# daigo0927/tf-raft

Hardware: AMD Instinct MI355X
Metric: image-pairs/sec at 448×512 iters_pred=24; final-iter EPE vs TF ref (higher is better)
Workload: dtype f32; 1 GPU; RAFT forward BASELINE configs[1]: batch 4/GPU 448x512 iters_pred=24 random weights; pairs_per_gpu=4, global_batch=4, parallelism=dp1, collective=none

## Files before the change

### include/raft_hip.h

```cpp
#ifndef RAFT_HIP_H_
#define RAFT_HIP_H_

#include <stddef.h>
#include <stdint.h>

#ifdef __cplusplus
extern "C" {
#endif

#define RAFT_HIP_VERSION 222
#define RAFT_MAX_LEVELS 4

enum {
    RAFT_OK = 0,
    RAFT_E_NULL = -1,
    RAFT_E_SHAPE = -2,
    RAFT_E_UNSUPPORTED = -3,
    RAFT_E_ALIGN = -4
};

int raft_version(void);
const char *raft_error_string(int rc);

int raft_set_option(const char *name, const char *value);
int raft_set_thread_concurrency(int n);
int raft_get_option(const char *name, char *buf, size_t len);

uint32_t raft_crc32c(uint32_t crc, const void *data, size_t n);


int raft_corr_pyramid_layout(int B, int h, int w, int levels,
                             int64_t *level_offsets ,
                             int *lh , int *lw );

int64_t raft_corr_build_workspace_floats(int B, int h, int w, int C, int levels);

int raft_corr_build_f32(const float *fmap1, const float *fmap2, int B, int h, int w, int C,
                        int levels, float *pyr, const int64_t *level_offsets,
                        float *workspace, void *stream);

int raft_corr_lookup_f32(const float *pyr, const int64_t *level_offsets, const float *coords,
                         int B, int h, int w, int levels, int radius,
                         float *out, int ld_out, void *stream);

int raft_fmap_pyramid_f32(const float *fmap2, int B, int h, int w, int C, int levels,
                          float *fmap2_pyr, void *stream);
int raft_corr_lookup_ondemand_f32(const float *fmap1, const float *fmap2_pyr,
                                  const float *coords, int B, int h, int w, int C,
                                  int levels, int radius, float *out, int ld_out,
                                  void *stream);

int raft_bilinear_sampler_f32(const float *image, const float *coords, int64_t n, int h, int w,
                              int kh, int kw, float *out, void *stream);

int raft_coords_grid_f32(float *coords, int B, int h, int w, void *stream);


int raft_upsample_convex_f32(const float *flow, const float *mask, int B, int h, int w,
                             float *out, void *stream);

int raft_upflow8_f32(const float *flow, int B, int h, int w, float *out, void *stream);

int raft_stream_copy_f32(const float *src, float *dst, int64_t n, void *stream);

int raft_crop_or_pad_f32(const float *src, float *dst, int N, int Hs, int Ws, int Ht, int Wt, int C, void *stream);
int raft_crop_or_pad_u8_f32(const uint8_t *src, float *dst, int N, int Hs, int Ws, int Ht, int Wt, int C, void *stream);
int raft_crop_or_pad_u8(const uint8_t *src, uint8_t *dst, int N, int Hs, int Ws, int Ht, int Wt, int C, void *stream);

int raft_resize_f32(const float *src, float *dst, int N, int Hs, int Ws, int Ht, int Wt, int C,
                    const int *y_first, const int *y_count, const float *y_weights, int y_max_taps,
                    const int *x_first, const int *x_count, const float *x_weights, int x_max_taps,
                    const float *chan_scale, void *stream);
int raft_resize_u8_f32(const uint8_t *src, float *dst, int N, int Hs, int Ws, int Ht, int Wt, int C,
                       const int *y_first, const int *y_count, const float *y_weights, int y_max_taps,
                       const int *x_first, const int *x_count, const float *x_weights, int x_max_taps,
                       const float *chan_scale, void *stream);

#define RAFT_TILE_MAX_PER_AXIS 32
#define RAFT_TILE_MAX_TAPS 4
typedef struct RaftTileOrigins {
    int32_t ny, nx;
    int32_t oy[RAFT_TILE_MAX_PER_AXIS];
    int32_t ox[RAFT_TILE_MAX_PER_AXIS];
} RaftTileOrigins;

int raft_tile_gather_f32(const float *src, float *dst, int N, int Hs, int Ws, int Ht, int Wt, int C, RaftTileOrigins origins,
                         void *stream);
int raft_tile_gather_u8_f32(const uint8_t *src, float *dst, int N, int Hs, int Ws, int Ht, int Wt, int C, RaftTileOrigins origins,
                            void *stream);

int raft_tile_blend_f32(const float *tiles, float *dst, int64_t M, int N, int H, int W, int Ht, int Wt, RaftTileOrigins origins,
                        const int *y_first, const int *y_count, const float *y_weights, int y_max_taps,
                        const int *x_first, const int *x_count, const float *x_weights, int x_max_taps, void *stream);

int64_t raft_flow_to_image_workspace_floats(int N);
int raft_flow_rad_max_f32(const float *flow, float *partial, int N, int Hs, int Ws, int Ht, int Wt, float clip, void *stream);
int raft_flow_to_image_u8(const float *flow, const float *partial, uint8_t *image, int N, int Hs, int Ws, int Ht, int Wt,
                          float clip, int bgr, float fixed_rad_max, void *stream);

int raft_warp_f32(const float *src, const float *flow, float *dst, uint8_t *inside, int N, int H, int W, int C, void *stream);
int raft_warp_u8_f32(const uint8_t *src, const float *flow, float *dst, uint8_t *inside, int N, int H, int W, int C, void *stream);
int raft_flow_consistency_f32(const float *flow_a, const float *flow_b, uint8_t *occluded_a, uint8_t *occluded_b, int N, int H, int W,
                              float alpha, float beta, void *stream);


typedef struct {
    double inv_fx, inv_fy;
    double fx, fy;
    double hue[2], sat[2], val[2];
    float alpha[2], beta[2];
    int32_t W1, H1;
    int32_t x0, y0;
    int32_t resize;
    int32_t flip_h, flip_v;
    int32_t color[2];
    int32_t n_rect;
    int32_t rect[2][4];
} RaftAugmentParams;

#define RAFT_AUGMENT_SUM_BLOCKS 64

int raft_augment_params_bytes(void);

int raft_augment_sums_u8(const uint8_t *img2, const RaftAugmentParams *params, uint32_t *partial, int N, int H, int W, void *stream);

int raft_augment_gather_u8(const uint8_t *img1, const uint8_t *img2, const float *flow, const RaftAugmentParams *params,
                           const uint32_t *partial, uint8_t *out1, uint8_t *out2, float *out_flow, float *valid,
                           int N, int H, int W, int h, int w, void *stream);

int raft_augment_gather_sparse_u8(const uint8_t *img1, const uint8_t *img2, const float *flow, const float *valid_in,
                                  const RaftAugmentParams *params, const uint32_t *partial, uint8_t *out1, uint8_t *out2,
                                  float *out_flow, float *valid_out, int N, int H, int W, int h, int w, void *stream);

int raft_mfma_probe_f32(float *out, int blocks, int iters, void *stream);



enum { RAFT_ACT_NONE = 0, RAFT_ACT_RELU = 1 };

int raft_conv2d_f32(const float *a0, int lda0, int c0, const float *a1, int lda1, int c1,
                    const float *wp, const float *bias, int B, int H, int W, int kh, int kw,
                    int npad, int nvalid, int act, float scale, float *out, int ldo,
                    void *stream);

int raft_conv2d_winograd_f32(const float *a0, int lda0, int c0, const float *a1, int lda1, int c1,
                             const float *wp, const float *bias, int B, int H, int W, int npad,
                             int nvalid, int act, float scale, float *out, int ldo, void *stream);

int raft_conv2d_winograd4_f32(const float *a0, int lda0, int c0, const float *a1, int lda1, int c1,
                              const float *wp, const float *bias, int B, int H, int W, int npad,
                              int nvalid, int act, float scale, float *out, int ldo, void *stream);

int raft_conv1d_winograd_f32(const float *a0, int lda0, int c0, const float *a1, int lda1, int c1,
                             const float *wp, const float *bias, int B, int H, int W, int kh, int kw,
                             int npad, int nvalid, int act, float scale, float *out, int ldo, void *stream);

int raft_conv1d_winograd4_f32(const float *a0, int lda0, int c0, const float *a1, int lda1, int c1,
                              const float *wp, const float *bias, int B, int H, int W, int kh, int kw,
                              int npad, int nvalid, int act, float scale, float *out, int ldo, void *stream);

int raft_lookup_convc1_f32(const float *pyr, const int64_t *level_offsets, const float *coords, int B, int h, int w,
                           const float *wp, const float *bias, int npad, int nvalid, float *out, int ldo, void *stream);


typedef struct raft_conv_weights {
    const float *wp;
    const float *bias;
    int npad;
} raft_conv_weights;

typedef struct raft_basic_update_weights {
    raft_conv_weights convc1, convc2, convf1, convf2, conv;
    raft_conv_weights gru_zr1, gru_q1, gru_zr2, gru_q2;
    raft_conv_weights fh1_mask0, fh2, mask2;
    raft_conv_weights gru_ctx1, gru_ctx2;
    raft_conv_weights convc2_w, convf2_w, conv_w, fh1_mask0_w;
    raft_conv_weights gru_zr1_w, gru_q1_w, gru_zr2_w, gru_q2_w;
    raft_conv_weights fh1_w;
    raft_conv_weights gru_zr1_w4, gru_q1_w4, gru_zr2_w4, gru_q2_w4;
    raft_conv_weights convc1_f;
    raft_conv_weights gru_ctx1_w4, gru_ctx2_w4;
    raft_conv_weights convc2_w44, conv_w44, fh1_mask0_w44, fh1_w44;
    raft_conv_weights convf2_w44;
} raft_basic_update_weights;

typedef struct raft_state {
    float *net, *x, *corr, *coords1, *flow, *delta, *mask, *ws, *ctx;
} raft_state;

int64_t raft_update_workspace_floats(int B, int h, int w);

int raft_prepare_state_f32(const float *cnet, int B, int h, int w, const raft_state *st,
                           void *stream);

int raft_gru_context_f32(const raft_basic_update_weights *wts, int B, int h, int w,
                         const raft_state *st, void *stream);

int raft_update_basic_f32(const raft_basic_update_weights *wts, int B, int h, int w,
                          const raft_state *st, void *stream);

int raft_iterate_basic_f32(const raft_basic_update_weights *wts, const float *pyr,
                           const int64_t *level_offsets, int B, int h, int w, int iters,
                           const raft_state *st, float *flow_up, void *stream);

typedef struct raft_loop_ctx raft_loop_ctx;
int raft_loop_ctx_create(raft_loop_ctx **ctx);
int raft_loop_ctx_destroy(raft_loop_ctx *ctx);

int raft_iterate_basic_overlap_f32(const raft_basic_update_weights *wts, const float *pyr,
                                   const int64_t *level_offsets, int B, int h, int w, int iters,
                                   const raft_state *st, float *flow_up, void *stream, void *aux0, void *aux1,
                                   raft_loop_ctx *ctx);

int raft_iterate_basic_ondemand_f32(const raft_basic_update_weights *wts, const float *fmap1,
                                    const float *fmap2_pyr, int C, int B, int h, int w, int iters,
                                    const raft_state *st, float *flow_up, void *stream, void *aux0, void *aux1,
                                    raft_loop_ctx *ctx);

int raft_iterate_basic_final_f32(const raft_basic_update_weights *wts, const float *pyr,
                                 const int64_t *level_offsets, int B, int h, int w, int iters,
                                 const raft_state *st, float *flow_up_last, void *stream, void *aux0, void *aux1,
                                 raft_loop_ctx *ctx);

#define RAFT_BASIC_STAGES 14
int raft_iterate_basic_timed_f32(const raft_basic_update_weights *wts, const float *pyr,
                                 const int64_t *level_offsets, int B, int h, int w, int iters,
                                 const raft_state *st, float *flow_up, void *stream,
                                 float *stage_ms );


enum { RAFT_NORM_NONE = 0, RAFT_NORM_INSTANCE = 1, RAFT_NORM_FOLDED = 2 };

typedef struct raft_encoder_weights {
    int c0, c1, c2, c3, cout, norm;
    raft_conv_weights conv1;
    raft_conv_weights block[6][3];
    raft_conv_weights conv2;
    const float *in_gamma[19];
    const float *in_beta[19];
    raft_conv_weights block_w[6][2];
    raft_conv_weights block_w44[6][2];
} raft_encoder_weights;

int64_t raft_encoder_workspace_floats(const raft_encoder_weights *w, int n, int H, int W);

int raft_encoder_f32(const raft_encoder_weights *w, const float *images, int n, int H, int W,
                     int input_affine, float *out, float *workspace, void *stream);
int raft_encoder_pair_f32(const raft_encoder_weights *w, const float *images_a, const float *images_b, int n_each, int H, int W,
                          int input_affine, float *out, float *workspace, void *stream);


typedef struct raft_small_update_weights {
    raft_conv_weights convc1, convf1, convf2, conv, gru_zr, gru_q, fh1, fh2;
    raft_conv_weights conv_w, gru_zr_w, gru_q_w, fh1_w;
} raft_small_update_weights;

int64_t raft_small_update_workspace_floats(int B, int h, int w);
int raft_prepare_state_small_f32(const float *cnet, int B, int h, int w, const raft_state *st,
                                 void *stream);
int raft_update_small_f32(const raft_small_update_weights *wts, int B, int h, int w,
                          const raft_state *st, void *stream);
int raft_iterate_small_f32(const raft_small_update_weights *wts, const float *pyr,
                           const int64_t *level_offsets, int B, int h, int w, int iters,
                           const raft_state *st, float *flow_up, void *stream);


int raft_forward_interpolate_f32(const float *flow, int B, int h, int w, float *out, void *stream);
int raft_warm_start_f32(const float *flow_init, int B, int h, int w, const raft_state *st, void *stream);
int raft_warm_start_small_f32(const float *flow_init, int B, int h, int w, const raft_state *st, void *stream);


int64_t raft_metrics_workspace_doubles(void);
int raft_flow_metrics_f32(const float *flow_gt, const unsigned char *valid, const float *flow_pred,
                          int64_t npix, float max_flow, float *out5, double *workspace, void *stream);
int raft_sequence_loss_f32(const float *flow_gt, const unsigned char *valid, const float *preds,
                           int64_t pred_stride, int n_predictions, int64_t npix, double gamma, float max_flow,
                           float *loss_out, double *workspace, void *stream);



int raft_sequence_loss_grad_f32(const float *flow_gt, const unsigned char *valid, const float *preds,
                                int64_t pred_stride, int n_predictions, int64_t npix, double gamma, float max_flow,
                                float upstream, float *d_preds, void *stream);

int64_t raft_photometric_loss_workspace_doubles(void);
int raft_photometric_loss_f32(const float *image1, const float *image2, const uint8_t *mask, const float *preds,
                              int64_t pred_stride, int n_predictions, int B, int H, int W, double gamma, float smooth_weight,
                              float edge_weight, float eps, float upstream, float *out3, float *d_preds, double *workspace,
                              void *stream);

int64_t raft_census_loss_workspace_bytes(int n_predictions, int B, int H, int W);
int raft_census_loss_f32(const float *image1, const float *image2, const uint8_t *mask, const float *preds, int64_t pred_stride,
                         int n_predictions, int B, int H, int W, double gamma, float census_weight, float upstream,
                         const float *add_to, float *out2, float *d_preds, int accumulate, void *workspace, void *stream);

int raft_corr_lookup_backward_f32(const float *pyr, const int64_t *level_offsets, const float *coords,
                                  const float *d_out, int ld_out, int B, int h, int w, int levels, int radius,
                                  float *d_coords, float *d_pyr, void *stream);

int raft_relu_backward_f32(const float *y, const float *dy, float *dx, int64_t n, void *stream);

int raft_pack_train_conv_f32(const float *kernel, const float *bias, int kh, int kw, int cin, int cout, int dgrad, int mode,
                             const double *g, int gt, int kpad, int npad, float *wp, float *bias_out, void *stream);

int64_t raft_conv2d_wgrad_workspace_floats(int cin, int cout, int B, int H, int W, int kh, int kw);
int raft_conv2d_wgrad_f32(const float *x, int ldx, int cin, const float *dy, int ldy, int cout, int B, int H, int W,
                          int kh, int kw, float *d_kernel, float *d_bias, float *workspace, void *stream);
int raft_conv2d_wgrad_multi_f32(const float *const *xs, const float *const *dys, int nseg, int ldx, int cin, int ldy, int cout,
                                int B, int H, int W, int kh, int kw, float *d_kernel, float *d_bias, float *workspace, void *stream);


int raft_conv7x7_c2_f32(const float *flow, const float *kernel, const float *bias, int cout, int B, int H, int W,
                        float *out, int ldo, void *stream);
int64_t raft_conv7x7_c2_wgrad_workspace_floats(int cout);
int raft_conv7x7_c2_backward_f32(const float *flow, const float *dy, int ldy, const float *kernel, int cout, int B, int H,
                                 int W, float *d_flow, float *d_kernel, float *d_bias, float *workspace, void *stream);

int raft_gru_gate_zr_f32(const float *a_zr, const float *h, int C, int64_t M, float *z, float *r, float *rh, void *stream);
int raft_gru_gate_q_f32(const float *a_q, const float *z, const float *h, int64_t n, float *q, float *h_new, void *stream);
int raft_gru_gate_q_backward_f32(const float *d_h_new, const float *z, const float *q, const float *h, int64_t n,
                                 float *dz_pre, float *dq_pre, float *dh, void *stream);
int raft_gru_gate_r_backward_f32(const float *d_rh, const float *r, const float *h, int64_t n, float *dr_pre, float *dh,
                                 void *stream);
int raft_axpby_f32(float alpha, const float *a, float beta, const float *b, float *out, int64_t n, void *stream);

int64_t raft_upsample_convex_backward_workspace_floats(int B, int h, int w);
int raft_upsample_convex_backward_f32(const float *flow, const float *mask, const float *d_up, int B, int h, int w,
                                      float *d_flow, float *d_mask, float *workspace, void *stream);

// ... 41 lines not shown
```

### tf_raft_amd/csrc/conv_wino1d.h

```cpp
#pragma once
#include <stdlib.h>

#include "conv_mfma.h"

#ifndef RAFT_WINO1D_ABL
#define RAFT_WINO1D_ABL 0
#endif

template <int AXIS, int TNW, int EPI, int TM, int MO>
__device__ __forceinline__ void wino1d_epilogue(const ConvArgs &p, f32x4 (&acc)[TM][MO + 4][TNW], int rbp, int cg, int G, int LR,
                                                int b, int y0, int x0, int n0, int M) {
    constexpr int TILE_H = AXIS == 0 ? 2 * TM : 2 * MO * TM, TILE_W = AXIS == 0 ? 16 * MO : 16;
    const EpiBuffers eb = raft_epi_buffers<EPI>(p, M);
    const __amdgpu_buffer_rsrc_t ri = raft_epi_init_buffer(p, M);
    const bool interior = (y0 + TILE_H <= p.H) & (x0 + TILE_W <= p.W);
#pragma unroll
    for (int i = 0; i < TM; ++i) {
        const int rb = TM * rbp + i;
        const int yb = AXIS == 0 ? y0 + rb : y0 + MO * rb;
        const int xb = AXIS == 0 ? x0 + MO * 4 * G : x0 + 4 * G;
        const unsigned pix0 = (unsigned)((b * p.H + yb) * p.W + xb);
        unsigned dead[4][MO];
#pragma unroll
        for (int r = 0; r < 4; ++r)
#pragma unroll
            for (int jx = 0; jx < MO; ++jx) {
                const int yy = AXIS == 0 ? yb : yb + jx;
                const int xx = AXIS == 0 ? xb + MO * r + jx : xb + r;
                dead[r][jx] = (interior | ((yy < p.H) & (xx < p.W))) ? 0u : RAFT_OOB;
            }
        auto es = [&](int r, int jx) { return AXIS == 0 ? MO * r + jx : jx * p.W + r; };
#pragma unroll
        for (int j = 0; j < TNW; ++j) {
            const int n = n0 + (cg * TNW + j) * 16 + LR;
            const EpiChannel<EPI> ch(p, n);
            const float bias = p.bias[n];
            f32x4 y[MO];
            if constexpr (MO == 2) {
                y[0] = ((acc[i][0][j] + acc[i][1][j]) + (acc[i][2][j] + acc[i][3][j])) + acc[i][4][j];
                y[1] = ((acc[i][1][j] - acc[i][2][j]) + 0.5f * (acc[i][3][j] - acc[i][4][j])) + acc[i][5][j];
            } else {
                const f32x4 s12 = acc[i][1][j] + acc[i][2][j], d12 = acc[i][1][j] - acc[i][2][j];
                const f32x4 s34 = acc[i][3][j] + acc[i][4][j], d34 = acc[i][3][j] - acc[i][4][j];
                const f32x4 s56 = acc[i][5][j] + acc[i][6][j], d56 = acc[i][5][j] - acc[i][6][j];
                y[0] = (acc[i][0][j] + s12) + (s34 + s56);
                y[1] = (d12 + 0.5f * d34) + 2.0f * d56;
                y[2] = (s12 + 0.25f * s34) + 4.0f * s56;
                y[3] = ((d12 + 0.125f * d34) + 8.0f * d56) + acc[i][7][j];
            }
            const EpiBases ba = raft_epi_bases<EPI>(p, ch, pix0);
            float iv[4][MO] = {}, hv[4][MO] = {}, zv[4][MO] = {};
#pragma unroll
            for (int r = 0; r < 4; ++r)
#pragma unroll
                for (int jx = 0; jx < MO; ++jx) {
                    if (RAFT_WINO1D_ABL & 8) {
                        iv[r][jx] = hv[r][jx] = zv[r][jx] = 0.5f;
                        continue;
                    }
                    iv[r][jx] = raft_buffer_load_f32(ri, ba.init | dead[r][jx], es(r, jx) * p.ldi * 4);
                    if (EPI == EPI_GRU_ZR || EPI == EPI_GRU_Q) hv[r][jx] = raft_buffer_load_f32(eb.e0, ba.e0 | dead[r][jx], es(r, jx) * p.lde0 * 4);
                    if (EPI == EPI_GRU_Q) zv[r][jx] = raft_buffer_load_f32(eb.e1, ba.e1 | dead[r][jx], es(r, jx) * p.lde1 * 4);
                }
#pragma unroll
            for (int r = 0; r < 4; ++r)
#pragma unroll
                for (int jx = 0; jx < MO; ++jx) {
                    const float v = (y[jx][r] + iv[r][jx]) + bias;
                    const int so0 = es(r, jx) * p.ldo0 * 4;
                    if ((RAFT_WINO1D_ABL & 8) && v != 12345.678f) continue;
                    if constexpr (EPI == EPI_GRU_ZR) {
                        float z, rh;
                        raft_epi_gate_zr(v, hv[r][jx], &z, &rh);
                        raft_buffer_store_f32(z, eb.o0, ba.o0 | dead[r][jx], so0);
                        raft_buffer_store_f32(rh, eb.o1, ba.o1 | dead[r][jx], es(r, jx) * p.ldo1 * 4);
                    } else {
                        raft_buffer_store_f32(raft_epi_act<EPI>(v, hv[r][jx], zv[r][jx], p.scale), eb.o0, ba.o0 | dead[r][jx], so0);
                    }
                }
        }
    }
}

template <int AXIS, int TNW, int EPI, int CK = 1, int TM = 2, int MO = 2>
__global__ void __launch_bounds__(256, 2) conv_wino1d_kernel(ConvArgs p) {
    static_assert(MO == 2 || (MO == 4 && CK == 2), "F(4,5) stages 32 channels per barrier");
    constexpr int NT = MO + 4;
    constexpr int PF = (TM * TNW == 1) ? 4 : 2;
    constexpr int RING = PF == 2 ? (NT == 6 ? 3 : 4) : NT;
    constexpr int TILE_H = AXIS == 0 ? 2 * TM : 2 * MO * TM, TILE_W = AXIS == 0 ? 16 * MO : 16;
    constexpr int HH = AXIS == 0 ? 2 * TM : TILE_H + 4, HWP = AXIS == 0 ? TILE_W + 4 : 16, HP = HH * HWP;
    constexpr bool SWZ = AXIS == 0 && MO == 4;
    constexpr int LDA = SWZ ? 32 : AXIS == 0 ? (CK == 1 ? 20 : 36) : (CK == 1 ? 24 : 40);
    constexpr int ROW = SWZ ? HWP * LDA + (HWP / 4) * 8 : HWP * LDA;
    constexpr int QS = 4 * CK;
    constexpr int NA = (HP * QS + 255) / 256;
    constexpr int A_BUF = HH * ROW + 4;
    constexpr int BN = 32 * TNW;
    static_assert(EPI == EPI_LINEAR || EPI == EPI_RELU || EPI == EPI_GRU_ZR || EPI == EPI_GRU_Q, "epilogue");
    __shared__ __attribute__((aligned(16))) float smem[2 * A_BUF];

    const int tid = threadIdx.x, lane = tid & 63, w = tid >> 6;
    const int G = lane >> 4, LR = lane & 15;
    const int rbp = w & 1, cg = w >> 1;
    const int tiles_x = (p.W + TILE_W - 1) / TILE_W, tiles_y = (p.H + TILE_H - 1) / TILE_H;
    const int ntn = p.npad / BN;
    const int M = p.B * p.H * p.W;

    const int bid = raft_xcd_remap(blockIdx.x, gridDim.x);
    const int mt = bid / ntn, nt = bid - mt * ntn;
    const int tx0 = mt % tiles_x, ty0 = (mt / tiles_x) % tiles_y, b = mt / (tiles_x * tiles_y);
    const int y0 = ty0 * TILE_H, x0 = tx0 * TILE_W;
    const int n0 = nt * BN;
    const int cin = p.c0 + p.c1;
    const int nst = cin / (16 * CK);

    const __amdgpu_buffer_rsrc_t rs0 = raft_stage_src0(p, M, p.c0), rs1 = raft_stage_src1(p, M);
    const __amdgpu_buffer_rsrc_t rsw = raft_stage_weights(p, NT, cin);

    int pix[NA], lds_off[NA];
    raft_stage_items<256, QS, HWP, HP>(tid, b, p.H, p.W, y0 - (AXIS == 1 ? 2 : 0), x0 - (AXIS == 0 ? 2 : 0), 1,
                                       [](int, int hy, int hx) { return (hy * ROW + hx * LDA) / 4 + (SWZ ? (hx >> 2) * 2 : 0); },
                                       HH * ROW / 4, pix, lds_off);
    f32x4 ra[NA];
    auto gload = [&](int c) { raft_stage_gload(p, rs0, rs1, pix, c * 16 * CK, tid % QS, ra); };
    auto lstore = [&](int buf) { raft_stage_lstore(smem + buf * A_BUF, lds_off, ra); };

    auto a_lane = [&](int i) {
        const int rb = TM * rbp + i;
        return (AXIS == 0 ? rb * ROW + MO * LR * LDA + (SWZ ? LR * 8 : 0) : (MO * rb * HWP + LR) * LDA) + G * 4;
    };
    auto koff = [](int k) { return AXIS == 0 ? k * LDA + (SWZ ? (k >> 2) * 8 : 0) : k * HWP * LDA; };
    const unsigned b_lane = raft_stage_b_lane(p, G, n0, cg * 16 * TNW, LR);
    f32x4 fb[RING][TNW];
    auto frag_b = [&](int c, int t, f32x4 *bf) { raft_stage_frag_b<TNW>(p, rsw, b_lane, cin, t, c * 4, bf); };
    auto transform = [&](int buf, int sub, int i, f32x4 *V) {
        const float *base = smem + buf * A_BUF + a_lane(i) + sub * 16;
        f32x4 d[NT];
#pragma unroll
        for (int k = 0; k < NT; ++k) d[k] = *(const f32x4 *)(base + koff(k));
        if constexpr (MO == 2) {
            const f32x4 s12 = d[1] + d[2], m12 = d[1] - d[2], s34 = d[3] + d[4], m34 = d[3] - d[4];
            const f32x4 a = d[3] - d[1], bb = d[4] - d[2];
            V[0] = (d[0] + 4.0f * d[4]) - 5.0f * d[2];
            V[1] = 4.0f * s34 - s12;
            V[2] = m12 - 4.0f * m34;
            V[3] = a + 2.0f * bb;
            V[4] = 2.0f * bb - a;
            V[5] = (d[1] + 4.0f * d[5]) - 5.0f * d[3];
        } else {
            const f32x4 s34 = d[3] + d[4], m34 = d[3] - d[4];
            const f32x4 pa = (4.0f * d[1] + d[5]) - 5.0f * d[3], qa = (4.0f * d[2] + d[6]) - 5.0f * d[4];
            const f32x4 pb = (d[1] + 4.0f * d[5]) - 5.0f * d[3], qb = (d[2] + 4.0f * d[6]) - 5.0f * d[4];
            V[0] = 4.0f * (d[6] - d[0]) + 21.0f * (d[2] - d[4]);
            V[1] = 4.0f * ((d[1] + d[2]) + (d[5] + d[6])) - 17.0f * s34;
            V[2] = 4.0f * ((d[2] - d[1]) + (d[6] - d[5])) + 17.0f * m34;
            V[3] = pa + 2.0f * qa;
            V[4] = 2.0f * qa - pa;
            V[5] = 2.0f * pb + qb;
            V[6] = qb - 2.0f * pb;
            V[7] = 4.0f * (d[7] - d[1]) + 21.0f * (d[3] - d[5]);
        }
    };

    f32x4 acc[TM][NT][TNW];
#pragma unroll
    for (int i = 0; i < TM; ++i)
#pragma unroll
        for (int t = 0; t < NT; ++t)
#pragma unroll
            for (int j = 0; j < TNW; ++j) acc[i][t][j] = f32x4{0.f, 0.f, 0.f, 0.f};

    gload(0);
#pragma unroll
    for (int t = 0; t < PF; ++t) frag_b(0, t, fb[t]);
    lstore(0);
    raft_barrier_lds();
    if (nst > 1) gload(1);
    for (int st = 0; st < nst; ++st) {
        const int buf = st & 1;
        const bool more = st + 1 < nst;
#pragma unroll
        for (int sub = 0; sub < CK; ++sub) {
            const int c = st * CK + sub;
            const bool more_c = more || sub + 1 < CK;
            f32x4 V[TM][NT];
#pragma unroll
            for (int i = 0; i < TM; ++i)
                if (!(RAFT_WINO1D_ABL & 2) || (st == 0 && sub == 0)) transform(buf, sub, i, V[i]);
            if (sub == CK - 1) {
                if (more && !(RAFT_WINO1D_ABL & 4)) {
                    lstore(buf ^ 1);
                    if (st + 2 < nst) gload(st + 2);
                }
                raft_barrier_lds();
            }
#pragma unroll
            for (int t = 0; t < NT; ++t) {
                if (RAFT_WINO1D_ABL & 1) {
                } else if (t + PF < NT)
                    frag_b(c, t + PF, fb[(t + PF) % RING]);
                else if (more_c)
                    frag_b(c + 1, t + PF - NT, fb[(t + PF) % RING]);
                __builtin_amdgcn_sched_barrier(0);
                if ((RAFT_WINO1D_ABL & 16) && t != 0) continue;
#pragma unroll
                for (int e = 0; e < 4; ++e)
#pragma unroll
                    for (int i = 0; i < TM; ++i)
#pragma unroll
                        for (int j = 0; j < TNW; ++j)
                            acc[i][t][j] = __builtin_amdgcn_mfma_f32_16x16x4f32(V[i][t][e], fb[t % RING][j][e], acc[i][t][j], 0, 0, 0);
            }
        }
    }

    wino1d_epilogue<AXIS, TNW, EPI, TM, MO>(p, acc, rbp, cg, G, LR, b, y0, x0, n0, M);
}
```

### tf_raft_amd/csrc/conv_wino1d.hip

```cpp
#include "conv_wino1d.h"

template <int AXIS, int TNW, int CK, int TM, int MO = 2>
static int launch_wino1d(const ConvArgs &a, int epi, int grid, hipStream_t s) {
    return raft_dispatch_epi<EPI_LINEAR, EPI_RELU, EPI_GRU_ZR, EPI_GRU_Q>(epi, [&](auto e) {
        conv_wino1d_kernel<AXIS, TNW, decltype(e)::value, CK, TM, MO><<<grid, 256, 0, s>>>(a);
        return raft_launch_status();
    });
}

template <int AXIS>
static int launch_wino1d_axis(const ConvArgs &a, int epi, int grid, Wino1dPlan p, hipStream_t s) {
    if (p.mo == 4) return p.tnw == 2 ? launch_wino1d<AXIS, 2, 2, 1, 4>(a, epi, grid, s) : launch_wino1d<AXIS, 1, 2, 1, 4>(a, epi, grid, s);
    if (p.tm == 2) {
        if (p.ck == 2) return p.tnw == 2 ? launch_wino1d<AXIS, 2, 2, 2>(a, epi, grid, s) : launch_wino1d<AXIS, 1, 2, 2>(a, epi, grid, s);
        return p.tnw == 2 ? launch_wino1d<AXIS, 2, 1, 2>(a, epi, grid, s) : launch_wino1d<AXIS, 1, 1, 2>(a, epi, grid, s);
    }
    if (p.ck == 2) return p.tnw == 2 ? launch_wino1d<AXIS, 2, 2, 1>(a, epi, grid, s) : launch_wino1d<AXIS, 1, 2, 1>(a, epi, grid, s);
    return p.tnw == 2 ? launch_wino1d<AXIS, 2, 1, 1>(a, epi, grid, s) : launch_wino1d<AXIS, 1, 1, 1>(a, epi, grid, s);
}

int raft_launch_conv_wino1d(const ConvArgs &a, int kh, int kw, int epi, hipStream_t s, Wino1dPlan p) {
    if (p.mo != 2 && p.mo != 4) return RAFT_E_UNSUPPORTED;
    if (p.mo == 4 && (a.c0 % 32 || a.c1 % 32)) return RAFT_E_UNSUPPORTED;
    if (!((kh == 1 && kw == 5) || (kh == 5 && kw == 1))) return RAFT_E_UNSUPPORTED;
    if (a.c0 <= 0 || a.c0 % 16 || a.c1 < 0 || a.c1 % 16 || a.npad <= 0 || a.npad % 32) return RAFT_E_UNSUPPORTED;
    RAFT_TRY(raft_check_operands(a, p.mo + 4, RAFT_CHECK_ALL));
    if (a.pre_scale || a.stats || (a.Hi && (a.Hi != a.H || a.Wi != a.W))) return RAFT_E_UNSUPPORTED;
    if (a.npad % (32 * p.tnw) || (p.ck == 2 && (a.c0 % 32 || a.c1 % 32))) return RAFT_E_UNSUPPORTED;
    const int grid = raft_wino1d_tiles(a.B, a.H, a.W, kh, p.mo, p.tm) * (a.npad / (32 * p.tnw));
    return kh == 5 ? launch_wino1d_axis<1>(a, epi, grid, p, s) : launch_wino1d_axis<0>(a, epi, grid, p, s);
}
```

### tf_raft_amd/csrc/host_util.hip

```cpp
#include <stddef.h>
#include <stdint.h>
#include <stdio.h>
#include <stdlib.h>
#include <string.h>

#include <atomic>
#include <mutex>

#include "common.h"

namespace {
struct Crc32cTable {
    uint32_t t[8][256];
    Crc32cTable() {
        for (uint32_t i = 0; i < 256; ++i) {
            uint32_t c = i;
            for (int k = 0; k < 8; ++k) c = (c >> 1) ^ (0x82f63b78u & (0u - (c & 1u)));
            t[0][i] = c;
        }
        for (uint32_t i = 0; i < 256; ++i)
            for (int s = 1; s < 8; ++s) t[s][i] = (t[s - 1][i] >> 8) ^ t[0][t[s - 1][i] & 0xffu];
    }
};
}

extern "C" uint32_t raft_crc32c(uint32_t crc, const void *data, size_t n) {
    static const Crc32cTable tab;
    const unsigned char *p = (const unsigned char *)data;
    uint32_t c = ~crc;
    while (n && ((uintptr_t)p & 7u)) {
        c = (c >> 8) ^ tab.t[0][(c ^ *p++) & 0xffu];
        --n;
    }
    while (n >= 8) {
        uint64_t w;
        __builtin_memcpy(&w, p, 8);
        w ^= c;
        c = tab.t[7][w & 0xff] ^ tab.t[6][(w >> 8) & 0xff] ^ tab.t[5][(w >> 16) & 0xff] ^ tab.t[4][(w >> 24) & 0xff] ^
            tab.t[3][(w >> 32) & 0xff] ^ tab.t[2][(w >> 40) & 0xff] ^ tab.t[1][(w >> 48) & 0xff] ^ tab.t[0][w >> 56];
        p += 8;
        n -= 8;
    }
    while (n--) c = (c >> 8) ^ tab.t[0][(c ^ *p++) & 0xffu];
    return ~c;
}

namespace {
const char *const kOptNames[RAFT_OPT_COUNT] = {
    "RAFT_CONV_WINO", "RAFT_SMALL_WINO", "RAFT_GRU_WINO", "RAFT_GRU_WINO4", "RAFT_WINO_TNW", "RAFT_WINO_SB",
    "RAFT_WINO_CK", "RAFT_WINO1D_TM",
    "RAFT_LOOKUP_FUSED", "RAFT_ONDEMAND_BLOCK", "RAFT_ENC_WINO",
    "RAFT_WINO_KS", "RAFT_CONV_WINO4", "RAFT_WINO4_KS", "RAFT_MASK_FUSED", "RAFT_ENC_WINO4", "RAFT_CONVC2_KS", "RAFT_CONVF2_KS",
    "RAFT_EVENT_FENCE", "RAFT_CORR_XCD", "RAFT_CORR_POOL",
};
constexpr int kTileEntries = 16;
struct TileRule {
    int npad, taps, code;
};
struct Options {
    std::atomic<int> val[RAFT_OPT_COUNT];
    std::atomic<bool> set[RAFT_OPT_COUNT];
    int env_val[RAFT_OPT_COUNT];
    bool env_set[RAFT_OPT_COUNT];
    std::mutex tile_mu;
    char tile_text[256], tile_env[256];
    TileRule tile_rules[kTileEntries];
    int n_tile_rules, tile_all;
    Options() {
        for (int i = 0; i < RAFT_OPT_COUNT; ++i) {
            const char *e = getenv(kOptNames[i]);
            env_set[i] = e && *e;
            env_val[i] = env_set[i] ? atoi(e) : 0;
            val[i].store(env_val[i]);
            set[i].store(env_set[i]);
        }
        const char *e = getenv("RAFT_CONV_TILE");
        snprintf(tile_env, sizeof(tile_env), "%s", e ? e : "");
        parse_tiles(tile_env);
    }
    void parse_tiles(const char *text) {
        snprintf(tile_text, sizeof(tile_text), "%s", text ? text : "");
        n_tile_rules = 0;
        tile_all = -1;
        if (!tile_text[0]) return;
        if (!strchr(tile_text, ':')) {
            tile_all = atoi(tile_text);
            return;
        }
        const char *p = tile_text;
        while (*p && n_tile_rules < kTileEntries) {
            TileRule r;
            if (sscanf(p, "%d:%d:%d", &r.npad, &r.taps, &r.code) == 3) tile_rules[n_tile_rules++] = r;
            p = strchr(p, ',');
            if (!p) break;
            ++p;
        }
    }
};
Options &opts() {
    static Options o;
    return o;
}
const int kOptsLoaded = (opts(), 0);
int opt_index(const char *name) {
    for (int i = 0; i < RAFT_OPT_COUNT; ++i)
        if (strcmp(name, kOptNames[i]) == 0) return i;
    return -1;
}
}

namespace {
thread_local int tl_concurrency = 1;
}
int raft_concurrency() { return tl_concurrency; }
extern "C" int raft_set_thread_concurrency(int n) {
    const int prev = tl_concurrency;
    tl_concurrency = n < 1 ? 1 : (n > 64 ? 64 : n);
    return prev;
}

int raft_opt(int id, int dflt) {
    Options &o = opts();
    return o.set[id].load(std::memory_order_relaxed) ? o.val[id].load(std::memory_order_relaxed) : dflt;
}
bool raft_opt_is_set(int id) { return opts().set[id].load(std::memory_order_relaxed); }

int raft_opt_conv_tile(int npad, int taps, bool (*valid)(int, int)) {
    Options &o = opts();
    std::lock_guard<std::mutex> g(o.tile_mu);
    if (o.tile_all >= 0) return valid(o.tile_all, npad) ? o.tile_all : -1;
    for (int i = 0; i < o.n_tile_rules; ++i) {
        const TileRule &r = o.tile_rules[i];
        if (r.npad == npad && r.taps == taps && valid(r.code, npad)) return r.code;
    }
    return -1;
}

extern "C" int raft_set_option(const char *name, const char *value) {
    RAFT_REQUIRE_PTR(name);
    Options &o = opts();
    if (strcmp(name, "RAFT_CONV_TILE") == 0) {
        std::lock_guard<std::mutex> g(o.tile_mu);
        o.parse_tiles(value ? value : o.tile_env);
        return RAFT_OK;
    }
    const int i = opt_index(name);
    if (i < 0) return RAFT_E_UNSUPPORTED;
    if (value == nullptr) {
        o.val[i].store(o.env_val[i]);
        o.set[i].store(o.env_set[i]);
    } else if (*value == 0) {
        o.set[i].store(false);
    } else {
        o.val[i].store(atoi(value));
        o.set[i].store(true);
    }
    return RAFT_OK;
}

extern "C" int raft_get_option(const char *name, char *buf, size_t len) {
    RAFT_REQUIRE_PTR(name);
    RAFT_REQUIRE_PTR(buf);
    RAFT_REQUIRE(len > 0, RAFT_E_SHAPE);
    Options &o = opts();
    if (strcmp(name, "RAFT_CONV_TILE") == 0) {
        std::lock_guard<std::mutex> g(o.tile_mu);
        snprintf(buf, len, "%s", o.tile_text);
        return RAFT_OK;
    }
    const int i = opt_index(name);
    if (i < 0) return RAFT_E_UNSUPPORTED;
    if (o.set[i].load())
        snprintf(buf, len, "%d", o.val[i].load());
    else
        buf[0] = 0;
    return RAFT_OK;
}
```

### tf_raft_amd/csrc/launch_plan.h

```cpp
#pragma once

#include <stdint.h>

#include "../../include/raft_hip.h"

enum RaftOptionId {
    RAFT_OPT_CONV_WINO, RAFT_OPT_SMALL_WINO, RAFT_OPT_GRU_WINO, RAFT_OPT_GRU_WINO4, RAFT_OPT_WINO_TNW, RAFT_OPT_WINO_SB,
    RAFT_OPT_WINO_CK, RAFT_OPT_WINO1D_TM,
    RAFT_OPT_LOOKUP_FUSED, RAFT_OPT_ONDEMAND_BLOCK, RAFT_OPT_ENC_WINO,
    RAFT_OPT_WINO_KS, RAFT_OPT_CONV_WINO4, RAFT_OPT_WINO4_KS, RAFT_OPT_MASK_FUSED, RAFT_OPT_ENC_WINO4, RAFT_OPT_CONVC2_KS, RAFT_OPT_CONVF2_KS,
    RAFT_OPT_EVENT_FENCE, RAFT_OPT_CORR_XCD, RAFT_OPT_CORR_POOL,
    RAFT_OPT_COUNT
};
int raft_opt(int id, int dflt);
bool raft_opt_is_set(int id);
int raft_opt_conv_tile(int npad, int taps, bool (*valid)(int code, int npad));

#ifdef __HIP__
#define RAFT_HOST_DEVICE __host__ __device__
#else
#define RAFT_HOST_DEVICE
#endif
RAFT_HOST_DEVICE static inline int raft_xcd_remap(int bid, int nwg) {
    const int xcd = bid & 7, q = nwg >> 3, r = nwg & 7;
    return (xcd < r ? xcd * (q + 1) : r * (q + 1) + (xcd - r) * q) + (bid >> 3);
}

enum RaftConvFamily { RAFT_FAM_HALO, RAFT_FAM_WINO, RAFT_FAM_WINO1D, RAFT_FAM_WINO4 };
struct HaloPlan { int th, tn; };
struct WinoPlan { int tnw, sb, ck, ks; };
struct Wino1dPlan { int mo, tnw, tm, ck; };
struct Wino4Plan { int ks; };
struct ConvChoice { int family; HaloPlan halo; WinoPlan wino; Wino1dPlan wino1d; Wino4Plan wino4; const raft_conv_weights *wt; };
typedef const raft_conv_weights *RaftWeights;
static inline ConvChoice raft_choice(HaloPlan p, RaftWeights wt = nullptr) { ConvChoice c = {RAFT_FAM_HALO}; c.halo = p; c.wt = wt; return c; }
static inline ConvChoice raft_choice(WinoPlan p, RaftWeights wt = nullptr) { ConvChoice c = {RAFT_FAM_WINO}; c.wino = p; c.wt = wt; return c; }
static inline ConvChoice raft_choice(Wino1dPlan p, RaftWeights wt = nullptr) { ConvChoice c = {RAFT_FAM_WINO1D}; c.wino1d = p; c.wt = wt; return c; }
static inline ConvChoice raft_choice(Wino4Plan p, RaftWeights wt = nullptr) { ConvChoice c = {RAFT_FAM_WINO4}; c.wino4 = p; c.wt = wt; return c; }

static inline bool raft_halo_code_valid(int code, int npad) {
    const int th = (code - 100) / 10, tn = (code - 100) % 10;
    return code >= 100 && (th == 4 || th == 7 || th == 8) && (tn == 1 || tn == 2) && npad % (64 * tn) == 0;
}

static inline HaloPlan raft_halo_plan(int B, int H, int W, int npad, int kh, int kw, int hint) {
    int code = raft_opt_conv_tile(npad, kh * kw, raft_halo_code_valid);
    if (code < 100) {
        static const int ths[3] = {4, 7, 8};
        double best = 1e30;
        code = 141;
        for (int ti = 0; ti < 3; ++ti)
            for (int tn = 1; tn <= 2; ++tn) {
                const int th = ths[ti];
                if (npad % (64 * tn)) continue;
                const int64_t blocks = (int64_t)B * ((H + th - 1) / th) * ((W + 15) / 16) * (npad / (64 * tn)) * hint;
                const int64_t per_cu = (blocks + 255) / 256;
                const int lds = 2 * ((th + kh - 1) * (16 + kw - 1) * 40 + 8) * 4;
                int resident = 160 * 1024 / lds;
                const int reg_limit = (tn == 2 && th >= 7) ? 1 : (th >= 7 ? 2 : 3);
                if (resident > reg_limit) resident = reg_limit;
                const int64_t conc = per_cu < resident ? per_cu : resident;
                const double pen = conc >= 3 ? 1.0 : (conc == 2 ? 1.05 : 1.15);
                const double eff = (th == 4 && kh * kw > 1) ? 0.88 : 1.0;
                const double cost = (double)per_cu * th * 16 * 64 * tn * pen / eff;
                if (cost < best) {
                    best = cost;
                    code = 100 + th * 10 + tn;
                }
            }
    }
    return {(code - 100) / 10, (code - 100) % 10};
}

static inline WinoPlan raft_wino_plan(int B, int H, int W, int c0, int c1, int npad, bool plain, int hint) {
    const int tiles = B * ((H + 3) / 4) * ((W + 31) / 32);
    const int forced = raft_opt(RAFT_OPT_WINO_TNW, 0);
    int tnw = (npad % 64 == 0 && (int64_t)tiles * (npad / 64) * hint >= 512) ? 2 : 1;
    if (forced == 1 || (forced == 2 && npad % 64 == 0)) tnw = forced;
    const int grid = tiles * (npad / (32 * tnw));
    const int sb = raft_opt(RAFT_OPT_WINO_SB, (tnw == 2 || grid <= 512) ? 1 : 0) != 0;
    const bool ck2_ok = c0 % 32 == 0 && c1 % 32 == 0;
    const bool ck2 = ck2_ok && raft_opt(RAFT_OPT_WINO_CK, grid <= 512 ? 2 : 1) == 2;
    const int ks = raft_opt(RAFT_OPT_WINO_KS, (tnw == 1 && grid * hint <= 224) ? 2 : 1);
    if (ks == 2 && tnw == 1 && ck2_ok && plain) {
        const bool ck4 = c0 % 64 == 0 && c1 % 64 == 0 && raft_opt(RAFT_OPT_WINO_CK, 4) == 4;
        return {1, 1, ck4 ? 4 : 2, 2};
    }
    return {tnw, sb, (tnw == 1 && ck2) ? 2 : 1, 1};
}

constexpr bool RAFT_WINO1D_CK2_DEFAULT = true;

static inline int raft_wino1d_tiles(int B, int H, int W, int kh, int mo, int tm) {
    if (mo == 4) return kh == 5 ? B * ((H + 7) / 8) * ((W + 15) / 16) : B * ((H + 1) / 2) * ((W + 63) / 64);
    return kh == 5 ? B * ((H + 4 * tm - 1) / (4 * tm)) * ((W + 15) / 16) : B * ((H + 2 * tm - 1) / (2 * tm)) * ((W + 31) / 32);
}

static inline Wino1dPlan raft_wino1d_plan(int B, int H, int W, int c0, int c1, int npad, int kh, int mo, int hint) {
    const int forced = raft_opt(RAFT_OPT_WINO_TNW, 0);
    const int tiles = raft_wino1d_tiles(B, H, W, kh, mo, 2);
    int tnw = (npad % 64 == 0 && (int64_t)tiles * (npad / 64) * hint >= 400) ? 2 : 1;
    if (forced == 1 || (forced == 2 && npad % 64 == 0)) tnw = forced;
    if (mo == 4) return {4, tnw, 1, 2};
    const int tm_forced = raft_opt(RAFT_OPT_WINO1D_TM, 0);
    const bool ck2 = c0 % 32 == 0 && c1 % 32 == 0 && raft_opt(RAFT_OPT_WINO_CK, RAFT_WINO1D_CK2_DEFAULT ? 2 : 1) == 2;
    int tm = (int64_t)tiles * (npad / (32 * tnw)) * hint >= 400 ? 2 : 1;
    if (tm_forced == 1 || tm_forced == 2) tm = tm_forced;
    return {2, tnw, tm, ck2 ? 2 : 1};
}

static inline Wino4Plan raft_wino4_plan(int B, int H, int W, int c0, int c1, int npad, bool plain, int hint, int layer_ks = 0) {
    const int grid1 = B * ((H + 7) / 8) * ((W + 63) / 64) * (npad / 64);
    int ks = raft_opt(RAFT_OPT_WINO4_KS, (layer_ks == 1 || layer_ks == 2) ? layer_ks : (grid1 * hint < 128 ? 2 : 1));
    if (ks != 2 || c0 % 32 || c1 % 32 || !plain) ks = 1;
    return {ks};
}

constexpr int RAFT_GRU_WINO_DEFAULT = 15;
constexpr int RAFT_GRU_WINO4_DEFAULT = 15;
constexpr int RAFT_WINO_DEFAULT = 13;
constexpr int RAFT_SMALL_WINO_DEFAULT = 15;
static inline int raft_wino4_default_mask(int64_t m) {
    return m < 2 * 3584 ? 0 : (8 | (m >= 3 * 3584 ? 1 | 2 : 0) | (m >= 8 * 3584 ? 4 : 0));
}

struct BasicLoopPlan {
    bool lookup_fused, mask_fused;
    ConvChoice convc1, convc2, convf2, conv, gru[4], fh1_mask0, fh1, mask2;
};

static inline BasicLoopPlan raft_basic_loop_plan(const raft_basic_update_weights &wt, int B, int h, int w, bool stored_volume, int hint) {
    BasicLoopPlan p = {};
    const int64_t m = (int64_t)B * h * w * hint;
    p.lookup_fused = stored_volume && wt.convc1_f.wp != nullptr && raft_opt(RAFT_OPT_LOOKUP_FUSED, 1) != 0;
    p.mask_fused = raft_opt(RAFT_OPT_MASK_FUSED, m >= 2 * 3584 ? 1 : 0) != 0 && wt.mask2.wp != nullptr && wt.mask2.npad == 576;
    p.convc1 = raft_choice(raft_halo_plan(B, h, w, wt.convc1.npad, 1, 1, hint), &wt.convc1);
    p.mask2 = raft_choice(raft_halo_plan(B, h, w, wt.mask2.npad, 1, 1, hint), &wt.mask2);

    const int wino = raft_opt(RAFT_OPT_CONV_WINO, RAFT_WINO_DEFAULT), wino4 = raft_opt(RAFT_OPT_CONV_WINO4, raft_wino4_default_mask(m));
    auto conv3x3 = [&](int bit, const raft_conv_weights &direct, const raft_conv_weights &w2, const raft_conv_weights &w44, int c0,
                       int layer_ks) {
        if (w44.wp != nullptr && (wino4 & bit)) return raft_choice(raft_wino4_plan(B, h, w, c0, 0, w44.npad, true, hint, layer_ks), &w44);
        if ((wino & bit) && w2.wp != nullptr) return raft_choice(raft_wino_plan(B, h, w, c0, 0, w2.npad, true, hint), &w2);
        return raft_choice(raft_halo_plan(B, h, w, direct.npad, 3, 3, hint), &direct);
    };
    p.convc2 = conv3x3(1, wt.convc2, wt.convc2_w, wt.convc2_w44, 256, raft_opt(RAFT_OPT_CONVC2_KS, 0));
    const int f2_grid1 = B * ((h + 7) / 8) * ((w + 63) / 64);
    p.convf2 = conv3x3(2, wt.convf2, wt.convf2_w, wt.convf2_w44, 128, raft_opt(RAFT_OPT_CONVF2_KS, f2_grid1 * hint >= 56 ? 1 : 0));
    p.conv = conv3x3(4, wt.conv, wt.conv_w, wt.conv_w44, 256, 0);
    p.fh1_mask0 = conv3x3(8, wt.fh1_mask0, wt.fh1_mask0_w, wt.fh1_mask0_w44, 128, 0);
    const int n4 = wt.fh1_mask0_w44.npad > 0 ? wt.fh1_mask0_w44.npad : wt.fh1_w44.npad;
    const int n2 = (wt.fh1_mask0_w.npad > 0 && wt.fh1_mask0_w.npad % 32 == 0) ? wt.fh1_mask0_w.npad : wt.fh1_w.npad;
    p.fh1 = wt.fh1_w44.wp != nullptr && (wino4 & 8) ? raft_choice(raft_wino4_plan(B, h, w, 128, 0, n4, true, hint), &wt.fh1_w44)
                                                    : raft_choice(raft_wino_plan(B, h, w, 128, 0, n2, true, hint), &wt.fh1_w);

    const int gmask = raft_opt(RAFT_OPT_GRU_WINO, RAFT_GRU_WINO_DEFAULT);
    const int gmask4 = raft_opt(RAFT_OPT_GRU_WINO4, m < 2 * 3584 ? 0 : RAFT_GRU_WINO4_DEFAULT);
    const raft_conv_weights *gw[4][3] = {{&wt.gru_zr1, &wt.gru_zr1_w, &wt.gru_zr1_w4}, {&wt.gru_q1, &wt.gru_q1_w, &wt.gru_q1_w4},
                                         {&wt.gru_zr2, &wt.gru_zr2_w, &wt.gru_zr2_w4}, {&wt.gru_q2, &wt.gru_q2_w, &wt.gru_q2_w4}};
    for (int l = 0; l < 4; ++l) {
        const int bit = 1 << l, kh = l < 2 ? 1 : 5, kw = 6 - kh;
        if ((gmask4 & bit) && gw[l][2]->wp != nullptr)
            p.gru[l] = raft_choice(raft_wino1d_plan(B, h, w, 128, 128, gw[l][2]->npad, kh, 4, hint), gw[l][2]);
        else if ((gmask & bit) && gw[l][1]->wp != nullptr)
            p.gru[l] = raft_choice(raft_wino1d_plan(B, h, w, 128, 128, gw[l][1]->npad, kh, 2, hint), gw[l][1]);
        else
            p.gru[l] = raft_choice(raft_halo_plan(B, h, w, gw[l][0]->npad, kh, kw, hint), gw[l][0]);
    }
    return p;
}

static inline ConvChoice raft_gru_ctx_plan(const raft_basic_update_weights &wt, int pass, int B, int h, int w, int hint) {
    const raft_conv_weights &w4 = pass == 0 ? wt.gru_ctx1_w4 : wt.gru_ctx2_w4;
    const int kh = pass == 0 ? 1 : 5;
    if (w4.wp != nullptr && (raft_opt(RAFT_OPT_GRU_WINO4, RAFT_GRU_WINO4_DEFAULT) & (pass == 0 ? 1 : 4)))
        return raft_choice(raft_wino1d_plan(B, h, w, 128, 0, w4.npad, kh, 4, hint), &w4);
    const raft_conv_weights &wc = pass == 0 ? wt.gru_ctx1 : wt.gru_ctx2;
    return raft_choice(raft_halo_plan(B, h, w, wc.npad, kh, 6 - kh, hint), &wc);
}

struct SmallLoopPlan { ConvChoice convc1, convf2, conv, gru_zr, gru_q, fh1; };

static inline SmallLoopPlan raft_small_loop_plan(const raft_small_update_weights &wt, int B, int h, int w, int hint) {
    SmallLoopPlan p = {};
    const int mask = raft_opt(RAFT_OPT_SMALL_WINO, RAFT_SMALL_WINO_DEFAULT);
    auto conv3x3 = [&](int bit, const raft_conv_weights &direct, const raft_conv_weights &w2, int c0, int c1) {
        return (mask & bit) && w2.wp != nullptr ? raft_choice(raft_wino_plan(B, h, w, c0, c1, w2.npad, true, hint), &w2)
                                                : raft_choice(raft_halo_plan(B, h, w, direct.npad, 3, 3, hint), &direct);
    };
    p.convc1 = raft_choice(raft_halo_plan(B, h, w, wt.convc1.npad, 1, 1, hint), &wt.convc1);
    p.convf2 = raft_choice(raft_halo_plan(B, h, w, wt.convf2.npad, 3, 3, hint), &wt.convf2);
    p.conv = conv3x3(1, wt.conv, wt.conv_w, 128, 0);
    p.gru_zr = conv3x3(2, wt.gru_zr, wt.gru_zr_w, 96, 160);
    p.gru_q = conv3x3(4, wt.gru_q, wt.gru_q_w, 96, 160);
    p.fh1 = conv3x3(8, wt.fh1, wt.fh1_w, 96, 0);
    return p;
}

static inline bool raft_enc_wino() { return raft_opt(RAFT_OPT_ENC_WINO, 1) != 0; }
static inline bool raft_enc_stage_wino4(int stage, int n, int Ho, int Wo, int F, int hint) {
    const int mask = raft_enc_wino() ? raft_opt(RAFT_OPT_ENC_WINO4, 7) : 0;
    return ((mask >> stage) & 1) &&
           (raft_opt_is_set(RAFT_OPT_ENC_WINO4) || (int64_t)n * ((Ho + 7) / 8) * ((Wo + 63) / 64) * ((F + 63) / 64) * hint > 256);
}
```

Baseline: 387.7 image-pairs/s.

## Split Winograd F(4,5) transform taps across wave pairs in wino1d kernel

Adds a tap-split variant of the 1-D Winograd F(4,5) convolution kernel. Each pair of waves handles half of the eight transform taps over a doubled set of output channels, then swaps partial accumulators through LDS before the shared epilogue. The goal is to spread per-wave transform and MFMA work and cut accumulator register pressure. The cost is an extra LDS exchange, two extra barriers, and more B-fragment loads per wave. It is on by default for the mo=4 path, with an option to turn it off and a plan-describe API.

```diff
diff --git a/include/raft_hip.h b/include/raft_hip.h
--- a/include/raft_hip.h
+++ b/include/raft_hip.h
@@ -25,6 +25,7 @@
 int raft_set_option(const char *name, const char *value);
 int raft_set_thread_concurrency(int n);
 int raft_get_option(const char *name, char *buf, size_t len);
+int raft_wino1d_plan_describe(int B, int H, int W, int npad, int kh, int mo, int *tnw, int *tm, int *ck, int *ts);
 
 uint32_t raft_crc32c(uint32_t crc, const void *data, size_t n);
 
diff --git a/tf_raft_amd/csrc/conv_wino1d.h b/tf_raft_amd/csrc/conv_wino1d.h
--- a/tf_raft_amd/csrc/conv_wino1d.h
+++ b/tf_raft_amd/csrc/conv_wino1d.h
@@ -82,9 +82,10 @@
     }
 }
 
-template <int AXIS, int TNW, int EPI, int CK = 1, int TM = 2, int MO = 2>
+template <int AXIS, int TNW, int EPI, int CK = 1, int TM = 2, int MO = 2, int TS = 1>
 __global__ void __launch_bounds__(256, 2) conv_wino1d_kernel(ConvArgs p) {
     static_assert(MO == 2 || (MO == 4 && CK == 2), "F(4,5) stages 32 channels per barrier");
+    static_assert(TS == 1 || (TS == 2 && MO == 4 && TM == 1), "the tap split is built for F(4,5) with one row block per wave");
     constexpr int NT = MO + 4;
     constexpr int PF = (TM * TNW == 1) ? 4 : 2;
     constexpr int RING = PF == 2 ? (NT == 6 ? 3 : 4) : NT;
@@ -163,6 +164,106 @@
         }
     };
 
+    if constexpr (TS == 2) {
+        constexpr int CB = 2 * TNW, HT = NT / 2;
+        constexpr int PF2 = TNW == 2 ? 1 : 2, RING2 = 2 * PF2;
+        static_assert(4 * HT * TNW * 256 <= 2 * A_BUF, "the accumulator exchange fits the staging buffers");
+        const int th = __builtin_amdgcn_readfirstlane(w >> 1);
+        const unsigned b_lane0 = raft_stage_b_lane(p, G, n0, 0, LR);
+        f32x4 accf[1][NT][TNW];
+        auto half = [&](auto thc) {
+            constexpr int TH = decltype(thc)::value;
+            auto tap_of = [](int h, int tl) { return h == 0 ? tl + 1 : (tl == 0 ? 0 : tl == 1 ? 7 : tl + 3); };
+            auto tap = [&](int tl) { return tap_of(TH, tl); };
+            f32x4 fh[RING2][CB];
+            auto frag_h = [&](int c, int tl, f32x4 *bf) { raft_stage_frag_b<CB>(p, rsw, b_lane0, cin, tap(tl), c * 4, bf); };
+            auto transform_h = [&](int buf, int sub, f32x4 *V) {
+                const float *base = smem + buf * A_BUF + a_lane(0) + sub * 16;
+                f32x4 d[NT];
+#pragma unroll
+                for (int k = TH == 0 ? 1 : 0; k < (TH == 0 ? NT - 1 : NT); ++k) d[k] = *(const f32x4 *)(base + koff(k));
+                if constexpr (TH == 0) {
+                    const f32x4 s34 = d[3] + d[4], m34 = d[3] - d[4];
+                    const f32x4 pa = (4.0f * d[1] + d[5]) - 5.0f * d[3], qa = (4.0f * d[2] + d[6]) - 5.0f * d[4];
+                    V[0] = 4.0f * ((d[1] + d[2]) + (d[5] + d[6])) - 17.0f * s34;
+                    V[1] = 4.0f * ((d[2] - d[1]) + (d[6] - d[5])) + 17.0f * m34;
+                    V[2] = pa + 2.0f * qa;
+                    V[3] = 2.0f * qa - pa;
+                } else {
+                    const f32x4 pb = (d[1] + 4.0f * d[5]) - 5.0f * d[3], qb = (d[2] + 4.0f * d[6]) - 5.0f * d[4];
+                    V[0] = 4.0f * (d[6] - d[0]) + 21.0f * (d[2] - d[4]);
+                    V[1] = 4.0f * (d[7] - d[1]) + 21.0f * (d[3] - d[5]);
+                    V[2] = 2.0f * pb + qb;
+                    V[3] = qb - 2.0f * pb;
+                }
+            };
+            f32x4 acc[HT][CB];
+#pragma unroll
+            for (int tl = 0; tl < HT; ++tl)
+#pragma unroll
+                for (int j = 0; j < CB; ++j) acc[tl][j] = f32x4{0.f, 0.f, 0.f, 0.f};
+
+            gload(0);
+#pragma unroll
+            for (int tl = 0; tl < PF2; ++tl) frag_h(0, tl, fh[tl]);
+            lstore(0);
+            raft_barrier_lds();
+            if (nst > 1) gload(1);
+            for (int st = 0; st < nst; ++st) {
+                const int buf = st & 1;
+                const bool more = st + 1 < nst;
+#pragma unroll
+                for (int sub = 0; sub < CK; ++sub) {
+                    const int c = st * CK + sub;
+                    const bool more_c = more || sub + 1 < CK;
+                    f32x4 V[HT];
+                    transform_h(buf, sub, V);
+                    if (sub == CK - 1) {
+                        if (more) {
+                            lstore(buf ^ 1);
+                            if (st + 2 < nst) gload(st + 2);
+                        }
+                        raft_barrier_lds();
+                    }
+#pragma unroll
+                    for (int tl = 0; tl < HT; ++tl) {
+                        if (tl + PF2 < HT)
+                            frag_h(c, tl + PF2, fh[(tl + PF2) % RING2]);
+                        else if (more_c)
+                            frag_h(c + 1, tl + PF2 - HT, fh[(tl + PF2) % RING2]);
+                        __builtin_amdgcn_sched_barrier(0);
+#pragma unroll
+                        for (int e = 0; e < 4; ++e)
+#pragma unroll
+                            for (int j = 0; j < CB; ++j)
+                                acc[tl][j] = __builtin_amdgcn_mfma_f32_16x16x4f32(V[tl][e], fh[tl % RING2][j][e], acc[tl][j], 0, 0, 0);
+                    }
+                }
+            }
+            raft_barrier_lds();
+            float *mine = smem + w * (HT * TNW * 256) + lane * 4;
+            const float *theirs = smem + (w ^ 2) * (HT * TNW * 256) + lane * 4;
+#pragma unroll
+            for (int tl = 0; tl < HT; ++tl)
+#pragma unroll
+                for (int j = 0; j < TNW; ++j) *(f32x4 *)(mine + (tl * TNW + j) * 256) = acc[tl][(1 - TH) * TNW + j];
+            raft_barrier_lds();
+#pragma unroll
+            for (int tl = 0; tl < HT; ++tl)
+#pragma unroll
+                for (int j = 0; j < TNW; ++j) {
+                    accf[0][tap(tl)][j] = acc[tl][TH * TNW + j];
+                    accf[0][tap_of(1 - TH, tl)][j] = *(const f32x4 *)(theirs + (tl * TNW + j) * 256);
+                }
+        };
+        if (th == 0)
+            half(std::integral_constant<int, 0>{});
+        else
+            half(std::integral_constant<int, 1>{});
+        wino1d_epilogue<AXIS, TNW, EPI, TM, MO>(p, accf, rbp, th, G, LR, b, y0, x0, n0, M);
+        return;
+    }
+
     f32x4 acc[TM][NT][TNW];
 #pragma unroll
     for (int i = 0; i < TM; ++i)
diff --git a/tf_raft_amd/csrc/conv_wino1d.hip b/tf_raft_amd/csrc/conv_wino1d.hip
--- a/tf_raft_amd/csrc/conv_wino1d.hip
+++ b/tf_raft_amd/csrc/conv_wino1d.hip
@@ -1,15 +1,17 @@
 #include "conv_wino1d.h"
 
-template <int AXIS, int TNW, int CK, int TM, int MO = 2>
+template <int AXIS, int TNW, int CK, int TM, int MO = 2, int TS = 1>
 static int launch_wino1d(const ConvArgs &a, int epi, int grid, hipStream_t s) {
     return raft_dispatch_epi<EPI_LINEAR, EPI_RELU, EPI_GRU_ZR, EPI_GRU_Q>(epi, [&](auto e) {
-        conv_wino1d_kernel<AXIS, TNW, decltype(e)::value, CK, TM, MO><<<grid, 256, 0, s>>>(a);
+        conv_wino1d_kernel<AXIS, TNW, decltype(e)::value, CK, TM, MO, TS><<<grid, 256, 0, s>>>(a);
         return raft_launch_status();
     });
 }
 
 template <int AXIS>
 static int launch_wino1d_axis(const ConvArgs &a, int epi, int grid, Wino1dPlan p, hipStream_t s) {
+    if (p.mo == 4 && p.ts == 1 && !RAFT_WINO1D_ABL)
+        return p.tnw == 2 ? launch_wino1d<AXIS, 2, 2, 1, 4, 2>(a, epi, grid, s) : launch_wino1d<AXIS, 1, 2, 1, 4, 2>(a, epi, grid, s);
     if (p.mo == 4) return p.tnw == 2 ? launch_wino1d<AXIS, 2, 2, 1, 4>(a, epi, grid, s) : launch_wino1d<AXIS, 1, 2, 1, 4>(a, epi, grid, s);
     if (p.tm == 2) {
         if (p.ck == 2) return p.tnw == 2 ? launch_wino1d<AXIS, 2, 2, 2>(a, epi, grid, s) : launch_wino1d<AXIS, 1, 2, 2>(a, epi, grid, s);
@@ -21,6 +23,7 @@
 
 int raft_launch_conv_wino1d(const ConvArgs &a, int kh, int kw, int epi, hipStream_t s, Wino1dPlan p) {
     if (p.mo != 2 && p.mo != 4) return RAFT_E_UNSUPPORTED;
+    if (p.ts != 0 && !(p.ts == 1 && p.mo == 4 && p.tm == 1)) return RAFT_E_UNSUPPORTED;
     if (p.mo == 4 && (a.c0 % 32 || a.c1 % 32)) return RAFT_E_UNSUPPORTED;
     if (!((kh == 1 && kw == 5) || (kh == 5 && kw == 1))) return RAFT_E_UNSUPPORTED;
     if (a.c0 <= 0 || a.c0 % 16 || a.c1 < 0 || a.c1 % 16 || a.npad <= 0 || a.npad % 32) return RAFT_E_UNSUPPORTED;
diff --git a/tf_raft_amd/csrc/host_util.hip b/tf_raft_amd/csrc/host_util.hip
--- a/tf_raft_amd/csrc/host_util.hip
+++ b/tf_raft_amd/csrc/host_util.hip
@@ -48,7 +48,7 @@
 namespace {
 const char *const kOptNames[RAFT_OPT_COUNT] = {
     "RAFT_CONV_WINO", "RAFT_SMALL_WINO", "RAFT_GRU_WINO", "RAFT_GRU_WINO4", "RAFT_WINO_TNW", "RAFT_WINO_SB",
-    "RAFT_WINO_CK", "RAFT_WINO1D_TM",
+    "RAFT_WINO_CK", "RAFT_WINO1D_TM", "RAFT_WINO1D_TS",
     "RAFT_LOOKUP_FUSED", "RAFT_ONDEMAND_BLOCK", "RAFT_ENC_WINO",
     "RAFT_WINO_KS", "RAFT_CONV_WINO4", "RAFT_WINO4_KS", "RAFT_MASK_FUSED", "RAFT_ENC_WINO4", "RAFT_CONVC2_KS", "RAFT_CONVF2_KS",
     "RAFT_EVENT_FENCE", "RAFT_CORR_XCD", "RAFT_CORR_POOL",
@@ -119,6 +119,18 @@
     return prev;
 }
 
+extern "C" int raft_wino1d_plan_describe(int B, int H, int W, int npad, int kh, int mo, int *tnw, int *tm, int *ck, int *ts) {
+    RAFT_REQUIRE_PTR(tnw);
+    RAFT_REQUIRE_PTR(tm);
+    RAFT_REQUIRE_PTR(ck);
+    RAFT_REQUIRE_PTR(ts);
+    RAFT_REQUIRE(B > 0 && H > 0 && W > 0 && npad > 0, RAFT_E_SHAPE);
+    if ((mo != 2 && mo != 4) || (kh != 1 && kh != 5) || npad % 32) return RAFT_E_UNSUPPORTED;
+    const Wino1dPlan p = raft_wino1d_plan(B, H, W, 128, 128, npad, kh, mo, raft_concurrency());
+    *tnw = p.tnw, *tm = p.tm, *ck = p.ck, *ts = p.ts;
+    return RAFT_OK;
+}
+
 int raft_opt(int id, int dflt) {
     Options &o = opts();
     return o.set[id].load(std::memory_order_relaxed) ? o.val[id].load(std::memory_order_relaxed) : dflt;
diff --git a/tf_raft_amd/csrc/launch_plan.h b/tf_raft_amd/csrc/launch_plan.h
--- a/tf_raft_amd/csrc/launch_plan.h
+++ b/tf_raft_amd/csrc/launch_plan.h
@@ -6,7 +6,7 @@
 
 enum RaftOptionId {
     RAFT_OPT_CONV_WINO, RAFT_OPT_SMALL_WINO, RAFT_OPT_GRU_WINO, RAFT_OPT_GRU_WINO4, RAFT_OPT_WINO_TNW, RAFT_OPT_WINO_SB,
-    RAFT_OPT_WINO_CK, RAFT_OPT_WINO1D_TM,
+    RAFT_OPT_WINO_CK, RAFT_OPT_WINO1D_TM, RAFT_OPT_WINO1D_TS,
     RAFT_OPT_LOOKUP_FUSED, RAFT_OPT_ONDEMAND_BLOCK, RAFT_OPT_ENC_WINO,
     RAFT_OPT_WINO_KS, RAFT_OPT_CONV_WINO4, RAFT_OPT_WINO4_KS, RAFT_OPT_MASK_FUSED, RAFT_OPT_ENC_WINO4, RAFT_OPT_CONVC2_KS, RAFT_OPT_CONVF2_KS,
     RAFT_OPT_EVENT_FENCE, RAFT_OPT_CORR_XCD, RAFT_OPT_CORR_POOL,
@@ -29,7 +29,7 @@
 enum RaftConvFamily { RAFT_FAM_HALO, RAFT_FAM_WINO, RAFT_FAM_WINO1D, RAFT_FAM_WINO4 };
 struct HaloPlan { int th, tn; };
 struct WinoPlan { int tnw, sb, ck, ks; };
-struct Wino1dPlan { int mo, tnw, tm, ck; };
+struct Wino1dPlan { int mo, tnw, tm, ck, ts; };
 struct Wino4Plan { int ks; };
 struct ConvChoice { int family; HaloPlan halo; WinoPlan wino; Wino1dPlan wino1d; Wino4Plan wino4; const raft_conv_weights *wt; };
 typedef const raft_conv_weights *RaftWeights;
@@ -90,6 +90,7 @@
 }
 
 constexpr bool RAFT_WINO1D_CK2_DEFAULT = true;
+constexpr int RAFT_WINO1D_TS_DEFAULT_TNW2 = 1, RAFT_WINO1D_TS_DEFAULT_TNW1 = 1;
 
 static inline int raft_wino1d_tiles(int B, int H, int W, int kh, int mo, int tm) {
     if (mo == 4) return kh == 5 ? B * ((H + 7) / 8) * ((W + 15) / 16) : B * ((H + 1) / 2) * ((W + 63) / 64);
@@ -101,12 +102,15 @@
     const int tiles = raft_wino1d_tiles(B, H, W, kh, mo, 2);
     int tnw = (npad % 64 == 0 && (int64_t)tiles * (npad / 64) * hint >= 400) ? 2 : 1;
     if (forced == 1 || (forced == 2 && npad % 64 == 0)) tnw = forced;
-    if (mo == 4) return {4, tnw, 1, 2};
+    if (mo == 4) {
+        const int ts = raft_opt(RAFT_OPT_WINO1D_TS, -1);
+        return {4, tnw, 1, 2, (ts == 0 || ts == 1) ? ts : (tnw == 2 ? RAFT_WINO1D_TS_DEFAULT_TNW2 : RAFT_WINO1D_TS_DEFAULT_TNW1)};
+    }
     const int tm_forced = raft_opt(RAFT_OPT_WINO1D_TM, 0);
     const bool ck2 = c0 % 32 == 0 && c1 % 32 == 0 && raft_opt(RAFT_OPT_WINO_CK, RAFT_WINO1D_CK2_DEFAULT ? 2 : 1) == 2;
     int tm = (int64_t)tiles * (npad / (32 * tnw)) * hint >= 400 ? 2 : 1;
     if (tm_forced == 1 || tm_forced == 2) tm = tm_forced;
-    return {2, tnw, tm, ck2 ? 2 : 1};
+    return {2, tnw, tm, ck2 ? 2 : 1, 0};
 }
 
 static inline Wino4Plan raft_wino4_plan(int B, int H, int W, int c0, int c1, int npad, bool plain, int hint, int layer_ks = 0) {
```

New measurement: 390.3 image-pairs/s, median of 6. Within noise of the previous version (+0.7%).
